# pacificclimate/VIC

Hardware: AMD Instinct MI355X
Metric: cell-timesteps/s (higher is better)
Workload: dtype f64

## Files before the change

vic_amd/csrc/vic_profile.hpp:

```cpp
#pragma once
#include "vic_surface.hpp"

namespace vic {

constexpr int NBUCKET = 2 * (VIC_MID_NODES + 2);
static_assert(NBUCKET <= 64, "one lane per work-list segment when the pending total is summed");

struct PArgs {
  const double* __restrict__ pin;
  const double* __restrict__ ts;
  double* __restrict__ pout;
  const int* __restrict__ pslot;
  const int* __restrict__ list;
  const int* __restrict__ count;
  int cap;
  int* next;
  int* count_zero;
  int* evalonly_zero;
  const int* pend_counts;
  const int* pend_eo;
  int* pend_out;
  int Nn, NOFLUX, EXP_TRANS, TFALLBACK;
  const int* jl;
};

__host__ __device__ inline int pout_stride(int Nn) { return Nn + 1 + (Nn + 1) / 2; }
__host__ __device__ inline int pout_hru_stride(int Nn) { return 2 * pout_stride(Nn) + 2; }
__host__ __device__ inline int pout_key(int Nn, int slot) { return 2 * pout_stride(Nn) + slot; }

constexpr int LOCKSTEP_GATE = 16;

constexpr double NODE_ROOT_RANGE = SOIL_DT + Brent::MAXTRIES * Brent::TSTEP;
constexpr double NODE_NEWTON_TOL = 1.e-8;
constexpr double NODE_PREDICT_TOL2 = 1.e-7;
constexpr int NODE_PREDICT_MAXIT = 12;
constexpr double NODE_NEWTON_ACCEPT = 2.e-11;
constexpr int NODE_NEWTON_MAXIT = 200;

struct NodeK {
  double AT0, B, C, D, EI, S, G, Y, EM, EMM;
  VIC_DEV void load(const double* __restrict__ r) {
    AT0 = r[PR_AT0]; B = r[PR_B]; C = r[PR_C]; D = r[PR_D]; EI = r[PR_EI]; S = r[PR_S]; G = r[PR_G]; Y = r[PR_Y];
    EM = r[PR_EMOIST]; EMM = r[PR_EMM];
// ... 156 lines not shown
    }
  }
  if (ok && !converged) {
    if (TFALLBACK) {
#pragma unroll
      for (int k = 0; k < NN; k++)
        if (k < Nn) { T[k] = T0[k]; cnt_add[k] += 1; }
      fbmask |= (Nn >= 32) ? 0xFFFFFFFFu : ((1u << Nn) - 1u);
    } else ok = false;
  }
}

VIC_DEV int profile_pick(const PArgs& a, const int* bcount, int slot) {
  int rem = slot, found = 0;
#pragma unroll 1
  for (int b = NBUCKET - 1; b >= 0; b--) {
    const int cb = bcount[b];
    if (rem < cb) { found = b * a.cap + rem; break; }
    rem -= cb;
  }
  return a.list[found];
}

constexpr int PROFILE_REG_WAVES = 2;
template <int NN, bool NEWTON>
__global__ __launch_bounds__(64) VIC_WAVES_PER_EU(PROFILE_REG_WAVES, PROFILE_REG_WAVES) void vic_profile_solve_reg(const PArgs a) {
  __shared__ int bcount[NBUCKET];
  __shared__ double T0l[NN * 64];
  __shared__ double Kl[3 * (NN - 2) * 64];
  const int lane = threadIdx.x;
#define T0(j) T0l[(j) * 64 + lane]
#define KL(f, j) Kl[((f) * (NN - 2) + (j) - 1) * 64 + lane]
  for (int b = lane; b < NBUCKET; b += 64) bcount[b] = a.count[b];
  if (blockIdx.x == 0) {
    for (int b = lane; b < NBUCKET; b += 64) a.count_zero[b] = 0;
    if (lane == 0) *a.evalonly_zero = 0;
    int v = (lane < NBUCKET) ? a.pend_counts[lane] : 0;
#pragma unroll
    for (int off = 32; off >= 1; off >>= 1) v += __shfl(v, lane ^ off);
    if (lane == 0) *a.pend_out = v + *a.pend_eo;
  }
  __syncthreads();
  int n = 0;
#pragma unroll
  for (int b = 0; b < NBUCKET; b++) n += bcount[b];
  if ((int)blockIdx.x * 64 >= n) return;

  constexpr int Nn = NN;
  const int jlast = a.NOFLUX ? Nn : Nn - 1;
  const int MAXIT = 1000;
  const double threshold = 1.e-2;
  const bool EXP_TRANS = a.EXP_TRANS != 0;

  bool have = false, sweeping = false, converged = false, ok = true, frozen_on = false;
  int hru = 0, ps = 0, it = 1, jl_lane = 0;
  unsigned fbmask = 0;
  int evcnt = 0;
  double T[NN];
  double kAT0[NN - 1], kB[NN - 1], kC[NN - 1], kD[NN - 1], kEI[NN - 1], kS[NN - 1], kEMM[NN - 1];
#pragma unroll
  for (int k = 0; k < NN; k++) T[k] = 0;
#pragma unroll
  for (int k = 0; k < NN - 1; k++) { kAT0[k] = 0; kB[k] = 0; kC[k] = 0; kD[k] = 0; kEI[k] = 0; kS[k] = 1; kEMM[k] = 0; }
// ... 101 lines not shown
      a.pout[(size_t)hru * pout_hru_stride(Nn) + pout_key(Nn, ps)] = T0(0);
      have = false;
    }
    PROF_ADD(24, t_fin);
  }
#undef T0
#undef KL
}

constexpr int LS_WAVES = 2;
template <int NN, bool NEWTON>
__global__ __launch_bounds__(64) VIC_WAVES_PER_EU(LS_WAVES, LS_WAVES) void vic_profile_solve_lockstep(const PArgs a) {
  using mask_t = typename NodeBound<NN>::mask_t;
  constexpr bool T0_LDS = NN <= VIC_MID_NODES;
  __shared__ int bcount[NBUCKET];
  __shared__ double Tl[NN * 64];
  __shared__ double T0l[T0_LDS ? NN * 64 : 1];
  const int lane = threadIdx.x;
#define T(j) Tl[(j) * 64 + lane]
#define T0(j) (T0_LDS ? T0l[(T0_LDS ? (j) : 0) * 64 + lane] : ((j) == 0 ? T0s : blk[(j) * PREC + PR_T0]))
  for (int b = lane; b < NBUCKET; b += 64) bcount[b] = a.count[b];
  if (blockIdx.x == 0) {
    for (int b = lane; b < NBUCKET; b += 64) a.count_zero[b] = 0;
    if (lane == 0) *a.evalonly_zero = 0;
    int v = (lane < NBUCKET) ? a.pend_counts[lane] : 0;
#pragma unroll
    for (int off = 32; off >= 1; off >>= 1) v += __shfl(v, lane ^ off);
    if (lane == 0) *a.pend_out = v + *a.pend_eo;
  }
  __syncthreads();
  int n = 0;
#pragma unroll
  for (int b = 0; b < NBUCKET; b++) n += bcount[b];
  if ((int)blockIdx.x * 64 >= n) return;

  const int Nn = node_count<NN>(a.Nn);
  const int jlast = a.NOFLUX ? Nn : Nn - 1;
  const int MAXIT = 1000;
  const double threshold = 1.e-2;
  const bool EXP_TRANS = a.EXP_TRANS != 0;

#define LS_REC() (a.pout + (size_t)hru * pout_hru_stride(Nn) + ps * pout_stride(Nn))
#define LS_CNT(j) (reinterpret_cast<int*>(LS_REC() + Nn + 1)[j])
  bool have = false, sweeping = false, converged = false, ok = true, frozen_on = false;
  int hru = 0, ps = 0, it = 1, jl_lane = 0;
  mask_t fbmask = 0;
  const double* __restrict__ blk = a.pin;
  double T0s = 0;
  bool more = true;
  while (true) {
    const unsigned long long idle = __ballot(!have);
// ... 103 lines not shown
```

vic_amd/csrc/vicgpu_api.hip:

```cpp
#include <hip/hip_runtime.h>
#include <stdio.h>
#include <stdlib.h>
#include <string.h>
#include <algorithm>
#include <atomic>
#include <chrono>
#include <memory>
#include <string>
#include <thread>
#include <vector>
#include "vicgpu.h"
#include <cstddef>
#include <type_traits>
#include "vic_glacier.hpp"
#include "vic_profile.hpp"
#include "vic_putdata.hpp"
#include "vic_host.hpp"

using namespace vic;

#define HIPIGN(call) do { hipError_t ign_ = (call); (void)ign_; } while (0)
#define HIPCHK(ctx, call)                                                                              \
  do {                                                                                                 \
    hipError_t e_ = (call);                                                                            \
// ... 42 lines not shown
  Dmy dmy;
  double* sd;
  int* si;
  double* flux;
  int* hru_err;
  const int* glist;
  int gcount;
  unsigned long long* ctx;
  double* pin;
  double* ts;
  double* pout;
  int* pslot;
  int* hstate;
  int* list;
  int* count;
  int list_cap;
  int* hkey;
  double* pimp;
  int* lastexp;
  int* jl;
  int phase;
};

constexpr int CTX_GROUP = 8, CTX_GROUP_B = 2;
constexpr size_t CTX_NA = sizeof(SurfSolve) / 8 + sizeof(SurfEBMut) / 8 + offsetof(SurfEBConst, Cs2) / 8;
constexpr size_t CTX_NA_PAD = (CTX_NA + CTX_GROUP - 1) / CTX_GROUP * CTX_GROUP;
constexpr size_t ctx_padded_words(size_t words) {
  return CTX_NA_PAD + ((words > CTX_NA ? words - CTX_NA : 0) + CTX_GROUP_B - 1) / CTX_GROUP_B * CTX_GROUP_B;
}
struct CtxRef {
  unsigned long long* p;
  int lane;
  VIC_DEV static CtxRef at(unsigned long long* base, size_t words_per_hru, size_t g) {
    return CtxRef{base + (g >> 6) * (ctx_padded_words(words_per_hru) * 64), (int)(g & 63)};
  }
  VIC_DEV unsigned long long* word(size_t W) const {
    if (W < CTX_NA) return p + (W / CTX_GROUP) * (64 * CTX_GROUP) + lane * CTX_GROUP + (W % CTX_GROUP);
    const size_t V = W - CTX_NA;
    return p + CTX_NA_PAD * 64 + (V / CTX_GROUP_B) * (64 * CTX_GROUP_B) + lane * CTX_GROUP_B + (V % CTX_GROUP_B);
  }
};
template <class T>
VIC_DEV void ctx_put(const CtxRef& r, size_t word0, const T& v) {
  static_assert(sizeof(T) % 8 == 0 && std::is_trivially_copyable<T>::value, "context structs are arrays of 8-byte words");
  constexpr int NW = sizeof(T) / 8;
  unsigned long long tmp[NW];
  __builtin_memcpy(tmp, &v, sizeof(T));
#pragma unroll
  for (int i = 0; i < NW; i++) *r.word(word0 + i) = tmp[i];
}
template <class T>
VIC_DEV void ctx_get(const CtxRef& r, size_t word0, T& v) {
  static_assert(sizeof(T) % 8 == 0 && std::is_trivially_copyable<T>::value, "context structs are arrays of 8-byte words");
  constexpr int NW = sizeof(T) / 8;
  unsigned long long tmp[NW];
#pragma unroll
  for (int i = 0; i < NW; i++) tmp[i] = *r.word(word0 + i);
  __builtin_memcpy(&v, tmp, sizeof(T));
}
constexpr int EBC_W_POST = offsetof(SurfEBConst, delta_t) / 8, EBC_W_ALWAYS = offsetof(SurfEBConst, ice0) / 8,
              EBC_W_FROZEN = offsetof(SurfEBConst, kappa_snow) / 8, EBC_W_SNOWCOV = offsetof(SurfEBConst, LongSnowIn) / 8,
              EBC_W_INCL = offsetof(SurfEBConst, lmoist) / 8, EBC_W_EVAP = offsetof(SurfEBConst, Wdew) / 8,
              EBC_W_CANOPY = offsetof(SurfEBConst, Cs2) / 8;
constexpr int EBM_W_FEED = offsetof(SurfEBMut, deltaCC) / 8, EBM_W_IN3 = offsetof(SurfEBMut, Tsnow_surf) / 8,
              EBM_W_TSNOW = offsetof(SurfEBMut, ra_used) / 8, EBM_W_RA1 = EBM_W_TSNOW + 1, EBM_W_VV = offsetof(SurfEBMut, vv) / 8,
              EBM_W_KEEP = offsetof(SurfEBMut, Tnew2) / 8;
static_assert(offsetof(SurfEBMut, fusion) / 8 == EBM_W_IN3 - 1 && offsetof(SurfEBMut, layerevap) / 8 == EBM_W_VV + 3, "SurfEBMut layout");
constexpr size_t CW_SV = sizeof(SurfSolve) / 8, CW_EBM = sizeof(SurfEBMut) / 8, CW_EBC = EBC_W_CANOPY,
                 CW_P = sizeof(SubStep) / 8, CW_L = sizeof(SubLoop) / 8, CW_C = sizeof(StepConst) / 8;
constexpr size_t CO_SV = 0, CO_EBM = CO_SV + CW_SV, CO_EBC = CO_EBM + CW_EBM, CO_P = CO_EBC + CW_EBC, CO_L = CO_P + CW_P,
                 CO_C = CO_L + CW_L, CO_W = CO_C + CW_C;
constexpr size_t CW_W = sizeof(WCarry) / 8, CO_WM = CO_W + CW_W;
template <int NN> constexpr size_t ctx_words() { return CO_WM + sizeof(WCarryMulti<NN>) / 8; }
static_assert(sizeof(StepConstPost) <= sizeof(StepConst), "StepConstPost is parked in StepConst's words");
static_assert(CTX_NA == CO_P, "region A of the context slab = what the evaluation kernel reads");
constexpr size_t CW_L_HEAD = offsetof(SubLoop, st_AlbedoOver) / 8;
constexpr size_t CW_SV_ITER = offsetof(SurfSolve, Tsurf) / 8;

template <class T>
VIC_DEV void ctx_put_words(const CtxRef& r, size_t word0, const T& v, int first, int last) {
  constexpr int NW = sizeof(T) / 8;
#pragma unroll
  for (int i = 0; i < NW; i++)
    if (i >= first && i < last) {
      unsigned long long w;
      __builtin_memcpy(&w, reinterpret_cast<const char*>(&v) + 8 * i, 8);
      *r.word(word0 + i) = w;
    }
}
template <class T>
VIC_DEV void ctx_get_words(const CtxRef& r, size_t word0, T& v, int first, int last) {
  constexpr int NW = sizeof(T) / 8;
#pragma unroll
  for (int i = 0; i < NW; i++)
    if (i >= first && i < last) {
      const unsigned long long w = *r.word(word0 + i);
      __builtin_memcpy(reinterpret_cast<char*>(&v) + 8 * i, &w, 8);
    }
}

// ... 596 lines not shown
  PROF_LANE(1);
}

struct EArgs {
  Opt o;
  LaunchMap map;
  int ncell, nhru, Nn;
  const int* glist;
  int gcount;
  const double* cell_params;
  const int* hpi;
  unsigned long long* ctx;
  size_t ctx_words;
  double* pout;
  int* pslot;
  double* ts;
  int* jl;
  int* hstate;
  int* list_next;
  int* count_next;
  int list_cap;
  const int* hkey;
  int* profile_next;
  int* evalonly;
  int* eo_list_next;
  int list_thr;
  const int* list_cur;
  const int* count_cur;
  const int* eo_list_cur;
  const int* npend_cur;
  int implicit;
  const double* veglib;
  const double* forcing;
  int month;
};

constexpr int EVAL_WAVES = 2;
__global__ __launch_bounds__(64) VIC_WAVES_PER_EU(EVAL_WAVES, EVAL_WAVES) void vic_surf_eval(const EArgs a) {
  if (blockIdx.x == 0 && threadIdx.x == 0) *a.profile_next = 0;
  const int npend = *a.npend_cur;
  int g;
  if (npend <= a.list_thr) {
    if ((int)blockIdx.x * 64 >= npend) return;
    __shared__ int bcount[NBUCKET];
    for (int b = threadIdx.x; b < NBUCKET; b += 64) bcount[b] = a.count_cur[b];
    __syncthreads();
    int nsolve = 0;
#pragma unroll 1
    for (int b = 0; b < NBUCKET; b++) nsolve += bcount[b];
    const int gi = blockIdx.x * 64 + threadIdx.x;
    if (gi >= npend) return;
    if (gi < nsolve) {
      int rem = gi, found = 0;
#pragma unroll 1
      for (int b = 0; b < NBUCKET; b++) {
        const int cb = bcount[b];
        if (rem < cb) { found = b * a.list_cap + rem; break; }
        rem -= cb;
      }
      g = a.list_cur[found];
    } else g = a.eo_list_cur[gi - nsolve];
  } else {
    const int gi = a.map.index(blockIdx.x, threadIdx.x, a.gcount);
    if (gi < 0) return;
    g = a.glist ? a.glist[gi] : gi;
  }
  const int hs = a.hstate[g];
  if ((hs & HS_STATE) != 1) return;
  const int cls = hs >> HS_CLS_SHIFT;
  const size_t nh = a.nhru;
  const int c = a.hpi[(size_t)HPI_CELL * nh + g];
  const int veg_idx = a.hpi[(size_t)HPI_VEG_INDEX * nh + g];
  const int ps = a.pslot[g];
  CellView cv{a.cell_params, a.ncell, c, a.o.Nnode, a.o.Nband};
  const Soil3 s3 = load_soil3(cv);
  SurfSolve sv;
  SurfEB eb;
  const CtxRef cx = CtxRef::at(a.ctx, a.ctx_words, g);
  ctx_get(cx, CO_SV, sv);
  ebc_get(cx, eb, cls);
  const bool is_final = sv.stage == SurfSolve::FINAL;
  const int slot = sv.on_record ? sv.final_slot : ps;
  {
    SurfEBMut& m = eb;
// ... 32 lines not shown
    a.pout[(size_t)g * pout_hru_stride(a.Nn) + pout_key(a.Nn, 1)] = NAN;
  }
  bool need_solve = sv.stage != SurfSolve::DONE;
  if (sv.stage == SurfSolve::FINAL && !a.implicit) {
    if (rec[pout_key(a.Nn, slot)] == sv.x) { sv.final_slot = slot; sv.on_record = 1; need_solve = false; }
    else if (rec[pout_key(a.Nn, slot ^ 1)] == sv.x) { sv.final_slot = slot ^ 1; sv.on_record = 1; need_solve = false; }
  }
  if (sv.stage == stage_before && (sv.stage == SurfSolve::ROOT || sv.stage == SurfSolve::ROOT_QUICK)) ctx_put_words(cx, CO_SV, sv, 0, (int)CW_SV_ITER);
  else ctx_put(cx, CO_SV, sv);
  if (sv.stage == SurfSolve::DONE) {
    const SurfEBMut& m = eb;
    if (at_root) {
      ctx_put_words(cx, CO_EBM, m, EBM_W_KEEP, (int)CW_EBM);
      ctx_put_words(cx, CO_EBM, m, EBM_W_TSNOW, EBM_W_TSNOW + 1);
      if (cls & EBG_FROZEN) ctx_put_words(cx, CO_EBM, m, EBM_W_IN3 - 1, EBM_W_IN3);
      if (cls & EBG_CANOPY) ctx_put_words(cx, CO_EBM, m, EBM_W_VV, EBM_W_VV + 6);
      else if (cls & EBG_EVAP) ctx_put_words(cx, CO_EBM, m, EBM_W_VV + 3, EBM_W_VV + 4);
    } else ctx_put(cx, CO_EBM, m);
  } else if (cls & EBG_INCL) ctx_put_words(cx, CO_EBM, static_cast<const SurfEBMut&>(eb), 0, EBM_W_FEED);
  if (sv.stage == SurfSolve::DONE) a.hstate[g] = 2;
  else if (need_solve) { a.ts[g] = sv.x; a.pslot[g] = slot ^ 1; }
  list_append(a.list_next, a.count_next, a.list_cap, need_solve, a.hkey[g], g);
  {
    const bool eo = sv.stage != SurfSolve::DONE && !need_solve;
    const unsigned long long m = __ballot(eo);
    if (m != 0) {
      const int lane = (int)__lane_id(), lead = __ffsll((long long)m) - 1;
      int base = 0;
      if (lane == lead) base = atomicAdd(a.evalonly, __popcll(m));
      base = __shfl(base, lead);
      if (eo) a.eo_list_next[base + __popcll(m & ((1ull << lane) - 1ull))] = g;
    }
  }
}

struct GArgs {
  Opt o;
  int ncell, nhru, reset;
  const double* cell_params;
  const int* cell_off;
  const int* cell_list;
  const int* hpi;
  double* sd;
  double* eq;
};

__global__ __launch_bounds__(64) void vic_glacier_fit(const GArgs a) {
  const int c = blockIdx.x * 64 + threadIdx.x;
  if (c >= a.ncell) return;
  const size_t nh = a.nhru, nc = a.ncell;
  CellView cv{a.cell_params, a.ncell, c, a.o.Nnode, a.o.Nband};
  double X[VIC_MAX_BANDS], Y[VIC_MAX_BANDS];
  int np = 0;
  for (int k = a.cell_off[c]; k < a.cell_off[c + 1]; k++) {
// ... 269 lines not shown
  I(VICGPU_SR_U(SRU_TFOLIAGE_FBCOUNT, Nn), SI_TFOLIAGE_FBCOUNT); I(VICGPU_SR_U(SRU_TSURF_FBCOUNT, Nn), SI_TSURF_FBCOUNT);
  I(VICGPU_SR_U(SRU_GLAC_SURF_TEMP_FBCOUNT, Nn), SI_GLAC_SURF_TEMP_FBCOUNT); I(VICGPU_SR_U(SRU_SNOW_SURF_TEMP_FBCOUNT, Nn), SI_SNOW_SURF_TEMP_FBCOUNT);
  I(VICGPU_SR_U(SRU_GLAC_SURF_TEMP_FBFLAG, Nn), SI_GLAC_SURF_TEMP_FBFLAG);
  F(VICGPU_SR_U(SRU_GLAC_VAPOR_FLUX, Nn), FX_GLAC_VAPOR_FLUX);
  if (GATHER) r[VICGPU_SR_U(SRU_SNOW_CANOPY_ALBEDO, Nn)] = 0.0;
  F(VICGPU_SR_U(SRU_SNOW_SURFACE_FLUX, Nn), FX_SNOW_SURFACE_FLUX);
  I(VICGPU_SR_U(SRU_SNOW_SURF_TEMP_FBFLAG, Nn), SI_SNOW_SURF_TEMP_FBFLAG);
  D(VICGPU_SR_U(SRU_SNOW_TMP_INT_STORAGE, Nn), SD_SNOW_TMP_INT_STORAGE);
  F(VICGPU_SR_U(SRU_SNOW_VAPOR_FLUX, Nn), FX_SNOW_VAPOR_FLUX);
#undef D
#undef I
#undef F
}

constexpr int RB_LAG = 3, RB_DEPTH = RB_LAG + 1;
struct FdChunk {
  int c0 = 0, ccount = 0;
  DevBuf<int> d_glist;
  int gcount = 0;
  LaunchMap map;
  DevBuf<int> d_list[2];
  DevBuf<int> d_fb_list, d_fb_count;
  DevBuf<int> d_count;
  DevBuf<int> d_elist[2];
  int list_cap = 0;
  PinnedBuf<int> h_count;
  Stream stream;
  Event done, readback[RB_DEPTH];
  std::string err;
  int status = 0;
  long long rounds = 0, steps = 0;
};

struct Domain {
  int ncell = 0, nhru = 0;
  bool domain_ready = false;
  bool any_glacier = false;
  DevBuf<double> d_cp, d_hpd, d_sd, d_flux, d_cell_out, d_accum;
  DevBuf<int> d_hpi, d_si, d_cell_off, d_cell_list, d_hru_err, d_cell_err;
  bool fd = false;
  DevBuf<unsigned long long> d_ctx;
  DevBuf<double> d_pin, d_ts, d_pout;
  DevBuf<int> d_hstate, d_pslot, d_hkey, d_lastexp, d_jl;
  DevBuf<double> d_pimp;
  std::vector<FdChunk> chunks;
  bool put_on = false;
  int out_nrow = 0;
  OutLayout out_lay;
// ... 10 lines not shown
  DevBuf<double> d_veglib;
  Domain dom;
  double* d_forcing = nullptr;
  unsigned char* d_snowflag = nullptr;
  std::vector<int> dmy;
  int chunk_steps = 0;
  struct ForcingSlot {
    DevBuf<double> d_f, d_raw;
    DevBuf<unsigned char> d_s;
    PinnedBuf<char> h_stage;
    std::vector<int> dmy;
    int nsteps = 0;
    Event uploaded;
    Event released;
    bool upload_pending = false, was_current = false;
  } slot[2];
  int cur = -1, staged = -1;
  Stream stream, copy_stream;
  std::vector<Event> ev;
  int ev_used = 0;
  int write_fluxes = 1;
  int steps_done = 0;
  int profile_waves = 0;
  int eval_list_pct = 30;
  bool node_newton = false;
  int ev_steps = 0;
  int out_step_ratio = 1;
};

static void free_domain(vicgpu_ctx* c) {
  c->dom = Domain();
  c->chunk_steps = 0;
  c->dmy.clear();
  c->cur = c->staged = -1;
  c->d_forcing = nullptr; c->d_snowflag = nullptr;
}

template <int NN>
static hipError_t launch_hru(const KArgs& ka, hipStream_t st, bool ordinary, bool glacier) {
  const int nblk = ka.map.nblocks(ka.gcount);
  if constexpr (NN == 3) {
    if (ordinary) hipLaunchKernelGGL((vic_hru_step<NN, false>), dim3(nblk), dim3(64), 0, st, ka);
  }
  if (glacier) hipLaunchKernelGGL((vic_hru_step<NN, true>), dim3(nblk), dim3(64), 0, st, ka);
  return hipGetLastError();
}

// ... 19 lines not shown
  if constexpr (NN == 10) {
    if (newton) hipLaunchKernelGGL((vic_profile_solve_reg<NN, true>), g, b, 0, st, pa);
    else hipLaunchKernelGGL((vic_profile_solve_reg<NN, false>), g, b, 0, st, pa);
  } else {
    if (newton) hipLaunchKernelGGL((vic_profile_solve_lockstep<NN, true>), g, b, 0, st, pa);
    else hipLaunchKernelGGL((vic_profile_solve_lockstep<NN, false>), g, b, 0, st, pa);
  }
  return hipGetLastError();
}

template <int NN>
static int profile_resident_waves(int device, bool newton) {
  int per_cu = 0, ncu = 0;
  hipError_t e;
  if constexpr (NN == 10) e = newton ? hipOccupancyMaxActiveBlocksPerMultiprocessor(&per_cu, vic_profile_solve_reg<NN, true>, 64, 0)
                                     : hipOccupancyMaxActiveBlocksPerMultiprocessor(&per_cu, vic_profile_solve_reg<NN, false>, 64, 0);
  else e = newton ? hipOccupancyMaxActiveBlocksPerMultiprocessor(&per_cu, vic_profile_solve_lockstep<NN, true>, 64, 0)
                  : hipOccupancyMaxActiveBlocksPerMultiprocessor(&per_cu, vic_profile_solve_lockstep<NN, false>, 64, 0);
  if (e != hipSuccess || per_cu <= 0) per_cu = 8;
  if (hipDeviceGetAttribute(&ncu, hipDeviceAttributeMultiprocessorCount, device) != hipSuccess || ncu <= 0) ncu = 256;
  return per_cu * ncu;
}

constexpr int CNT_LIST_STRIDE = 64, CNT_CURSOR = 128, CNT_EVALONLY = 160, CNT_EVALONLY_STRIDE = 32, CNT_NPEND = 224, CNT_TOTAL = 256;
static_assert(NBUCKET <= CNT_LIST_STRIDE, "counter block layout");
static inline int* cnt_list(int* d_count, int l) { return d_count + l * CNT_LIST_STRIDE; }
static inline int* cnt_evalonly(int* d_count, int l) { return d_count + CNT_EVALONLY + l * CNT_EVALONLY_STRIDE; }

static int fd_read_count(FdChunk* ch, int which, int* nsolve, int* nevalonly) {
  HIPCHK(ch, hipMemcpyAsync(ch->h_count, ch->d_count, sizeof(int) * CNT_TOTAL, hipMemcpyDeviceToHost, ch->stream));
  HIPCHK(ch, hipStreamSynchronize(ch->stream));
  int n = 0;
  for (int b = 0; b < NBUCKET; b++) n += ch->h_count[which * CNT_LIST_STRIDE + b];
  *nsolve = n;
  *nevalonly = ch->h_count[CNT_EVALONLY + which * CNT_EVALONLY_STRIDE];
  return VICGPU_OK;
}

#define NODE_DISPATCH(Nnode, F, ...)                                                                                          \
  (node_bound(Nnode) == 10 ? F<10>(__VA_ARGS__)                                                                           \
                           : node_bound(Nnode) == VIC_MID_NODES ? F<VIC_MID_NODES>(__VA_ARGS__) : F<VIC_MAX_NODES>(__VA_ARGS__))

static int fd_step(vicgpu_ctx* c, FdChunk* ch, KArgs ka) {
  const int Nn = c->o.Nnode;
  hipStream_t st = ch->stream;
  if (c->dom.any_glacier) HIPCHK(ch, NODE_DISPATCH(Nn, launch_hru, ka, st, false, true));
  HIPCHK(ch, hipMemsetAsync(ch->d_count, 0, sizeof(int) * CNT_TOTAL, st));
  int cur = 0;
  ka.phase = 0; ka.list = ch->d_list[cur]; ka.count = cnt_list(ch->d_count, cur); ka.list_cap = ch->list_cap;
  HIPCHK(ch, NODE_DISPATCH(Nn, launch_fd_stage, ka, c->o.NF > 1, st));
  PArgs pa;
  pa.pin = c->dom.d_pin; pa.ts = c->dom.d_ts; pa.pout = c->dom.d_pout; pa.pslot = c->dom.d_pslot; pa.Nn = Nn; pa.NOFLUX = c->o.NOFLUX; pa.EXP_TRANS = c->o.EXP_TRANS;
  pa.TFALLBACK = c->o.TFALLBACK; pa.next = ch->d_count + CNT_CURSOR; pa.cap = ch->list_cap; pa.jl = c->dom.d_jl;
  EArgs ea;
  ea.o = c->o; ea.ncell = c->dom.ncell; ea.nhru = c->dom.nhru; ea.Nn = Nn; ea.glist = ch->d_glist; ea.gcount = ch->gcount; ea.map = ch->map;
  ea.cell_params = c->dom.d_cp; ea.hpi = c->dom.d_hpi; ea.ctx = c->dom.d_ctx;
  ea.ctx_words = NODE_DISPATCH(Nn, ctx_words);
  ea.pout = c->dom.d_pout; ea.pslot = c->dom.d_pslot; ea.ts = c->dom.d_ts; ea.hstate = c->dom.d_hstate; ea.profile_next = ch->d_count + CNT_CURSOR;
  ea.list_thr = (int)((long long)ch->gcount * c->eval_list_pct / 100);
  ea.list_cap = ch->list_cap; ea.hkey = c->dom.d_hkey; ea.implicit = c->o.IMPLICIT; ea.jl = c->dom.d_jl;
  ea.veglib = c->d_veglib; ea.forcing = ka.forcing; ea.month = ka.dmy.month;
  const bool trace_rounds = getenv("VICGPU_TRACE_ROUNDS") != nullptr;
  const int FREE_ROUNDS = 6;
  const int nsub = c->o.NF;
  for (int p = 1; p <= nsub; p++) {
    int nmax = ch->gcount;
    int npend = -1;
    int rb_list[RB_DEPTH];
    int rb_first = -1;
    for (int round = 0;; round++) {
      pa.list = ch->d_list[cur]; pa.count = cnt_list(ch->d_count, cur); pa.count_zero = cnt_list(ch->d_count, cur ^ 1);
      pa.evalonly_zero = cnt_evalonly(ch->d_count, cur ^ 1);
      pa.pend_counts = cnt_list(ch->d_count, cur); pa.pend_eo = cnt_evalonly(ch->d_count, cur); pa.pend_out = ch->d_count + CNT_NPEND;
      if (c->o.IMPLICIT) {
        HIPCHK(ch, hipMemsetAsync(ch->d_fb_count, 0, sizeof(int) * (NBUCKET + 1), st));
        IArgs ia;
        ia.ncell = c->dom.ncell; ia.nhru = c->dom.nhru; ia.Nband = c->o.Nband; ia.pimp = c->dom.d_pimp; ia.hpi = c->dom.d_hpi; ia.cell_params = c->dom.d_cp;
        ia.hkey = c->dom.d_hkey; ia.fb_list = ch->d_fb_list; ia.fb_count = ch->d_fb_count; ia.lastexp = c->dom.d_lastexp; ia.cursor = ch->d_fb_count + NBUCKET;
        {
          int nblk = (nmax + 63) / 64;
          if (nblk > 4096) nblk = 4096;
          if (nblk < 1) nblk = 1;
          hipLaunchKernelGGL(vic_profile_solve_implicit, dim3(nblk), dim3(64), 0, st, pa, ia);
        }
        HIPCHK(ch, hipGetLastError());
        pa.list = ch->d_fb_list; pa.count = ch->d_fb_count;
      }
      HIPCHK(ch, NODE_DISPATCH(Nn, launch_profile, pa, nmax, c->profile_waves, c->node_newton, st));
      ea.list_next = ch->d_list[cur ^ 1]; ea.count_next = cnt_list(ch->d_count, cur ^ 1);
      ea.evalonly = cnt_evalonly(ch->d_count, cur ^ 1); ea.eo_list_next = ch->d_elist[cur ^ 1];
      ea.list_cur = ch->d_list[cur]; ea.count_cur = cnt_list(ch->d_count, cur);
      ea.eo_list_cur = ch->d_elist[cur]; ea.npend_cur = ch->d_count + CNT_NPEND;
      const bool sparse = npend >= 0 && npend <= ea.list_thr;
      hipLaunchKernelGGL(vic_surf_eval, dim3(sparse ? ((npend + 63) / 64 > 0 ? (npend + 63) / 64 : 1) : ea.map.nblocks(ch->gcount)), dim3(64), 0, st, ea);
      HIPCHK(ch, hipGetLastError());
      cur ^= 1;
      ch->rounds++;
      if (trace_rounds) {
        int n = 0, ne = 0;
        if (fd_read_count(ch, cur, &n, &ne) != VICGPU_OK) return VICGPU_ERR_HIP;
        fprintf(stderr, "vicgpu rounds: chunk %d sub-step %d round %d leaves %d solves + %d evaluation-only of %d\n", (int)(ch - &c->dom.chunks[0]), p, round, n, ne, ch->gcount);
      }
      if (round + 2 >= FREE_ROUNDS) {
        const int slot = round % RB_DEPTH;
        if (rb_first < 0) rb_first = round;
        HIPCHK(ch, hipMemcpyAsync(ch->h_count + slot * CNT_TOTAL, ch->d_count, sizeof(int) * CNT_TOTAL, hipMemcpyDeviceToHost, st));
        HIPCHK(ch, hipEventRecord(ch->readback[slot], st));
        rb_list[slot] = cur;
      }
      if (rb_first >= 0 && round - RB_LAG >= rb_first) {
        const int slot = (round - RB_LAG) % RB_DEPTH;
        HIPCHK(ch, hipEventSynchronize(ch->readback[slot]));
        const int* h = ch->h_count + slot * CNT_TOTAL;
        int n = 0;
        for (int b = 0; b < NBUCKET; b++) n += h[rb_list[slot] * CNT_LIST_STRIDE + b];
        const int neo = h[CNT_EVALONLY + rb_list[slot] * CNT_EVALONLY_STRIDE];
        if (n == 0 && neo == 0) break;
        nmax = n;
        npend = n + neo;
      }
    }
    ka.phase = p; ka.list = ch->d_list[cur]; ka.count = cnt_list(ch->d_count, cur);
    HIPCHK(ch, NODE_DISPATCH(Nn, launch_fd_stage, ka, c->o.NF > 1, st));
    if (p < nsub) {
      int n = 0, ne = 0;
      const int r = fd_read_count(ch, cur, &n, &ne);
      if (r != VICGPU_OK) return r;
      if (n == 0) break;
    }
  }
  ch->steps++;
  return VICGPU_OK;
}

static hipError_t launch_put_data(const vicgpu_ctx* c, hipStream_t st, int c0, int ccount, int s) {
  OArgs a;
  a.o = c->o; a.lay = c->dom.out_lay; a.ncell = c->dom.ncell; a.nhru = c->dom.nhru; a.c0 = c0; a.ccount = ccount;
  a.rec = s < 0 ? -1 : 0; a.out_step_ratio = c->out_step_ratio;
  a.cell_off = c->dom.d_cell_off; a.cell_list = c->dom.d_cell_list; a.cell_params = c->dom.d_cp; a.veglib = c->d_veglib;
  a.hpi = c->dom.d_hpi; a.hpd = c->dom.d_hpd; a.sd = c->dom.d_sd; a.si = c->dom.d_si; a.flux = c->dom.d_flux;
  a.forcing = s < 0 ? nullptr : c->d_forcing + (size_t)s * VIC_NFORCE * (c->o.NR + 1) * c->dom.ncell;
  a.cell_out = c->dom.d_cell_out; a.out_data = c->dom.d_out_data; a.out_agg = c->dom.d_out_agg; a.pb = c->dom.d_pb;
// ... 231 lines not shown
      ch.c0 = (int)((long long)ncell * k / nchunk);
      ch.ccount = (int)((long long)ncell * (k + 1) / nchunk) - ch.c0;
      std::vector<int> gl(cell_hru_list + cell_hru_offset[ch.c0], cell_hru_list + cell_hru_offset[ch.c0 + ch.ccount]);
      std::sort(gl.begin(), gl.end());
      ch.gcount = (int)gl.size();
      ch.map = LaunchMap();
      if (ch.ccount > 0 && ch.gcount % ch.ccount == 0 && !getenv("VICGPU_NO_XCD_MAP")) {
        const int nslot = ch.gcount / ch.ccount;
        bool regular = true;
        for (int sl = 0; sl < nslot && regular; sl++)
          for (int i = 0; i < ch.ccount; i++)
            if (gl[(size_t)sl * ch.ccount + i] != sl * ncell + ch.c0 + i || hpi[(size_t)HPI_CELL * nhru + gl[(size_t)sl * ch.ccount + i]] != ch.c0 + i) {
              regular = false;
              break;
            }
        if (regular) { ch.map.nslot = nslot; ch.map.ccount = ch.ccount; }
      }
      const size_t gn = ch.gcount > 0 ? ch.gcount : 1;
      HIPCHK(c, ch.d_glist.alloc(gn));
      ch.list_cap = ch.gcount > 0 ? ch.gcount : 1;
      HIPCHK(c, ch.d_list[0].alloc(gn * NBUCKET));
      HIPCHK(c, ch.d_list[1].alloc(gn * NBUCKET));
      HIPCHK(c, ch.d_count.alloc(CNT_TOTAL));
      HIPCHK(c, ch.d_elist[0].alloc(gn));
      HIPCHK(c, ch.d_elist[1].alloc(gn));
      if (c->o.IMPLICIT) {
        HIPCHK(c, ch.d_fb_list.alloc(gn * NBUCKET));
        HIPCHK(c, ch.d_fb_count.alloc(NBUCKET + 1));
      }
      HIPCHK(c, ch.h_count.alloc((size_t)CNT_TOTAL * RB_DEPTH));
      if (ch.gcount) HIPCHK(c, copy_on(c->stream, ch.d_glist, gl.data(), sizeof(int) * ch.gcount, hipMemcpyHostToDevice));
      HIPCHK(c, ch.stream.create());
      HIPCHK(c, ch.done.create(hipEventDisableTiming));
      for (Event& e : ch.readback) HIPCHK(c, e.create(hipEventDisableTiming));
    }
  }
  return VICGPU_OK;
}

int vicgpu_set_domain(vicgpu_ctx* c, int ncell, int nhru, const double* cell_params, const int* hpi, const double* hpd,
                      const int* cell_hru_offset, const int* cell_hru_list) {
  if (!c) return VICGPU_ERR_ARG;
  const int r = set_domain_impl(c, ncell, nhru, cell_params, hpi, hpd, cell_hru_offset, cell_hru_list);
  if (r == VICGPU_OK) c->dom.domain_ready = true;
  else if (r == VICGPU_ERR_HIP || r == VICGPU_ERR_NOMEM) {
    HIPIGN(hipSetDevice(c->device));
    free_domain(c);
  }
// ... 623 lines not shown
```

Measured before the change: 3.853 million.

## Stripe pending-HRU work list and regroup context slab by access class

Replaces the single global evaluation-only counter and split solve/eval-only lookup with a single pending list spread over 64 per-block stripes. The profile kernel builds a prefix sum over the stripe counts, and the sparse evaluation kernel finds each entry by binary search. This is meant to reduce atomic contention on one counter and simplify index lookup. It also permutes the region-A context words so that fields read together sit in the same sectors. The sparse-list threshold rises from 30% to 75% and is disabled in round 0. Costs include more counter memory, a larger host readback and a 64-entry reduction on the host.

```diff
diff --git a/vic_amd/csrc/vic_profile.hpp b/vic_amd/csrc/vic_profile.hpp
--- a/vic_amd/csrc/vic_profile.hpp
+++ b/vic_amd/csrc/vic_profile.hpp
@@ -5,6 +5,7 @@
 
 constexpr int NBUCKET = 2 * (VIC_MID_NODES + 2);
 static_assert(NBUCKET <= 64, "one lane per work-list segment when the pending total is summed");
+constexpr int PEND_STRIPES = 64, PEND_CNT_STRIDE = 32;
 
 struct PArgs {
   const double* __restrict__ pin;
@@ -16,9 +17,10 @@
   int cap;
   int* next;
   int* count_zero;
-  int* evalonly_zero;
   const int* pend_counts;
-  const int* pend_eo;
+  const int* pend_stripes;
+  int* pend_stripes_zero;
+  int* pend_prefix;
   int* pend_out;
   int Nn, NOFLUX, EXP_TRANS, TFALLBACK;
   const int* jl;
@@ -221,6 +223,22 @@
   return a.list[found];
 }
 
+static_assert(PEND_STRIPES == 64, "one lane per stripe");
+VIC_DEV void pend_pack(const PArgs& a, int lane, int keyed_total) {
+  a.pend_stripes_zero[lane * PEND_CNT_STRIDE] = 0;
+  const int cnt = a.pend_stripes[lane * PEND_CNT_STRIDE];
+  int incl = cnt;
+#pragma unroll
+  for (int off = 1; off < 64; off <<= 1) {
+    const int up = __shfl(incl, lane >= off ? lane - off : lane);
+    if (lane >= off) incl += up;
+  }
+  a.pend_prefix[lane + 1] = incl;
+  if (lane == 0) a.pend_prefix[0] = 0;
+  const int total = __shfl(incl, 63);
+  if (lane == 0) *a.pend_out = total > 0 ? total : keyed_total;
+}
+
 constexpr int PROFILE_REG_WAVES = 2;
 template <int NN, bool NEWTON>
 __global__ __launch_bounds__(64) VIC_WAVES_PER_EU(PROFILE_REG_WAVES, PROFILE_REG_WAVES) void vic_profile_solve_reg(const PArgs a) {
@@ -233,11 +251,10 @@
   for (int b = lane; b < NBUCKET; b += 64) bcount[b] = a.count[b];
   if (blockIdx.x == 0) {
     for (int b = lane; b < NBUCKET; b += 64) a.count_zero[b] = 0;
-    if (lane == 0) *a.evalonly_zero = 0;
     int v = (lane < NBUCKET) ? a.pend_counts[lane] : 0;
 #pragma unroll
     for (int off = 32; off >= 1; off >>= 1) v += __shfl(v, lane ^ off);
-    if (lane == 0) *a.pend_out = v + *a.pend_eo;
+    pend_pack(a, lane, v);
   }
   __syncthreads();
   int n = 0;
@@ -385,11 +402,10 @@
   for (int b = lane; b < NBUCKET; b += 64) bcount[b] = a.count[b];
   if (blockIdx.x == 0) {
     for (int b = lane; b < NBUCKET; b += 64) a.count_zero[b] = 0;
-    if (lane == 0) *a.evalonly_zero = 0;
     int v = (lane < NBUCKET) ? a.pend_counts[lane] : 0;
 #pragma unroll
     for (int off = 32; off >= 1; off >>= 1) v += __shfl(v, lane ^ off);
-    if (lane == 0) *a.pend_out = v + *a.pend_eo;
+    pend_pack(a, lane, v);
   }
   __syncthreads();
   int n = 0;
diff --git a/vic_amd/csrc/vicgpu_api.hip b/vic_amd/csrc/vicgpu_api.hip
--- a/vic_amd/csrc/vicgpu_api.hip
+++ b/vic_amd/csrc/vicgpu_api.hip
@@ -88,42 +88,6 @@
   int phase;
 };
 
-constexpr int CTX_GROUP = 8, CTX_GROUP_B = 2;
-constexpr size_t CTX_NA = sizeof(SurfSolve) / 8 + sizeof(SurfEBMut) / 8 + offsetof(SurfEBConst, Cs2) / 8;
-constexpr size_t CTX_NA_PAD = (CTX_NA + CTX_GROUP - 1) / CTX_GROUP * CTX_GROUP;
-constexpr size_t ctx_padded_words(size_t words) {
-  return CTX_NA_PAD + ((words > CTX_NA ? words - CTX_NA : 0) + CTX_GROUP_B - 1) / CTX_GROUP_B * CTX_GROUP_B;
-}
-struct CtxRef {
-  unsigned long long* p;
-  int lane;
-  VIC_DEV static CtxRef at(unsigned long long* base, size_t words_per_hru, size_t g) {
-    return CtxRef{base + (g >> 6) * (ctx_padded_words(words_per_hru) * 64), (int)(g & 63)};
-  }
-  VIC_DEV unsigned long long* word(size_t W) const {
-    if (W < CTX_NA) return p + (W / CTX_GROUP) * (64 * CTX_GROUP) + lane * CTX_GROUP + (W % CTX_GROUP);
-    const size_t V = W - CTX_NA;
-    return p + CTX_NA_PAD * 64 + (V / CTX_GROUP_B) * (64 * CTX_GROUP_B) + lane * CTX_GROUP_B + (V % CTX_GROUP_B);
-  }
-};
-template <class T>
-VIC_DEV void ctx_put(const CtxRef& r, size_t word0, const T& v) {
-  static_assert(sizeof(T) % 8 == 0 && std::is_trivially_copyable<T>::value, "context structs are arrays of 8-byte words");
-  constexpr int NW = sizeof(T) / 8;
-  unsigned long long tmp[NW];
-  __builtin_memcpy(tmp, &v, sizeof(T));
-#pragma unroll
-  for (int i = 0; i < NW; i++) *r.word(word0 + i) = tmp[i];
-}
-template <class T>
-VIC_DEV void ctx_get(const CtxRef& r, size_t word0, T& v) {
-  static_assert(sizeof(T) % 8 == 0 && std::is_trivially_copyable<T>::value, "context structs are arrays of 8-byte words");
-  constexpr int NW = sizeof(T) / 8;
-  unsigned long long tmp[NW];
-#pragma unroll
-  for (int i = 0; i < NW; i++) tmp[i] = *r.word(word0 + i);
-  __builtin_memcpy(&v, tmp, sizeof(T));
-}
 constexpr int EBC_W_POST = offsetof(SurfEBConst, delta_t) / 8, EBC_W_ALWAYS = offsetof(SurfEBConst, ice0) / 8,
               EBC_W_FROZEN = offsetof(SurfEBConst, kappa_snow) / 8, EBC_W_SNOWCOV = offsetof(SurfEBConst, LongSnowIn) / 8,
               EBC_W_INCL = offsetof(SurfEBConst, lmoist) / 8, EBC_W_EVAP = offsetof(SurfEBConst, Wdew) / 8,
@@ -139,9 +103,95 @@
 constexpr size_t CW_W = sizeof(WCarry) / 8, CO_WM = CO_W + CW_W;
 template <int NN> constexpr size_t ctx_words() { return CO_WM + sizeof(WCarryMulti<NN>) / 8; }
 static_assert(sizeof(StepConstPost) <= sizeof(StepConst), "StepConstPost is parked in StepConst's words");
-static_assert(CTX_NA == CO_P, "region A of the context slab = what the evaluation kernel reads");
 constexpr size_t CW_L_HEAD = offsetof(SubLoop, st_AlbedoOver) / 8;
 constexpr size_t CW_SV_ITER = offsetof(SurfSolve, Tsurf) / 8;
+
+constexpr int CTX_GROUP = 8, CTX_GROUP_B = 2;
+constexpr size_t CTX_NA = sizeof(SurfSolve) / 8 + sizeof(SurfEBMut) / 8 + offsetof(SurfEBConst, Cs2) / 8;
+static_assert(CTX_NA == CO_P, "region A of the context slab = what the evaluation kernel reads");
+constexpr int CTXR_ITER = 0, CTXR_COMMON = 16, CTXR_CLASS = 48, CTXR_SNOW = 64, CTXR_COLD = 72, CTXR_END = 104;
+struct CtxMap { unsigned char slab[CTX_NA]; int end[6]; };
+constexpr int ctx_map_run(CtxMap& m, int at, size_t first, size_t last) {
+  for (size_t w = first; w < last; w++) m.slab[w] = (unsigned char)at++;
+  return at;
+}
+constexpr CtxMap ctx_make_map() {
+  CtxMap m{};
+  int at = ctx_map_run(m, CTXR_ITER, CO_SV, CO_SV + CW_SV_ITER);
+  m.end[0] = at;
+  at = ctx_map_run(m, CTXR_COMMON, CO_EBM + EBM_W_FEED, CO_EBM + EBM_W_TSNOW);
+  at = ctx_map_run(m, at, CO_EBM + EBM_W_RA1, CO_EBM + EBM_W_RA1 + 1);
+  at = ctx_map_run(m, at, CO_EBC, CO_EBC + EBC_W_ALWAYS);
+  m.end[1] = at;
+  at = ctx_map_run(m, CTXR_CLASS, CO_EBC + EBC_W_ALWAYS, CO_EBC + EBC_W_FROZEN);
+  at = ctx_map_run(m, at, CO_EBC + EBC_W_INCL, CO_EBC + EBC_W_CANOPY);
+  m.end[2] = at;
+  at = ctx_map_run(m, CTXR_SNOW, CO_EBC + EBC_W_FROZEN, CO_EBC + EBC_W_INCL);
+  m.end[3] = at;
+  at = ctx_map_run(m, CTXR_COLD, CO_SV + CW_SV_ITER, CO_SV + CW_SV);
+  m.end[4] = at;
+  at = ctx_map_run(m, at, CO_EBM + EBM_W_TSNOW, CO_EBM + EBM_W_TSNOW + 1);
+  at = ctx_map_run(m, at, CO_EBM, CO_EBM + EBM_W_FEED);
+  at = ctx_map_run(m, at, CO_EBM + EBM_W_VV, CO_EBM + CW_EBM);
+  m.end[5] = at;
+  return m;
+}
+constexpr CtxMap CTX_MAP = ctx_make_map();
+constexpr bool ctx_map_is_permutation() {
+  bool used[CTXR_END] = {};
+  for (size_t w = 0; w < CTX_NA; w++) {
+    if (CTX_MAP.slab[w] >= CTXR_END || used[CTX_MAP.slab[w]]) return false;
+    used[CTX_MAP.slab[w]] = true;
+  }
+  int n = 0;
+  for (int i = 0; i < CTXR_END; i++) n += used[i] ? 1 : 0;
+  return n == (int)CTX_NA;
+}
+static_assert(ctx_map_is_permutation(), "parking map of region A");
+static_assert(CTXR_ITER % CTX_GROUP == 0 && CTXR_COMMON % CTX_GROUP == 0 && CTXR_CLASS % CTX_GROUP == 0 && CTXR_SNOW % CTX_GROUP == 0
+              && CTXR_COLD % CTX_GROUP == 0 && CTXR_END % CTX_GROUP == 0, "every range of the parking map starts on a sector boundary");
+static_assert(CTX_MAP.end[0] == CTXR_COMMON && CTX_MAP.end[1] <= CTXR_CLASS && CTX_MAP.end[2] <= CTXR_SNOW && CTX_MAP.end[3] <= CTXR_COLD
+              && CTX_MAP.end[4] <= CTXR_COLD + CTX_GROUP && CTX_MAP.end[5] <= CTXR_END && CTXR_END - CTX_MAP.end[5] < CTX_GROUP,
+              "ranges of the parking map; the tail of SurfSolve, which every evaluation fetches, in one sector");
+static_assert(CTX_MAP.end[1] - CTXR_COMMON == 31 && CTX_MAP.end[2] - CTXR_CLASS == 13,
+              "the iteration's inputs: 4 sectors for every class, 2 more for frozen soil / evaporation / canopy");
+constexpr size_t CTX_NA_PAD = CTXR_END;
+constexpr size_t ctx_padded_words(size_t words) {
+  return CTX_NA_PAD + ((words > CTX_NA ? words - CTX_NA : 0) + CTX_GROUP_B - 1) / CTX_GROUP_B * CTX_GROUP_B;
+}
+struct CtxRef {
+  unsigned long long* p;
+  int lane;
+  VIC_DEV static CtxRef at(unsigned long long* base, size_t words_per_hru, size_t g) {
+    return CtxRef{base + (g >> 6) * (ctx_padded_words(words_per_hru) * 64), (int)(g & 63)};
+  }
+  VIC_DEV unsigned long long* word(size_t W) const {
+    if (W < CTX_NA) {
+      const size_t S = CTX_MAP.slab[W];
+      return p + (S / CTX_GROUP) * (64 * CTX_GROUP) + lane * CTX_GROUP + (S % CTX_GROUP);
+    }
+    const size_t V = W - CTX_NA;
+    return p + CTX_NA_PAD * 64 + (V / CTX_GROUP_B) * (64 * CTX_GROUP_B) + lane * CTX_GROUP_B + (V % CTX_GROUP_B);
+  }
+};
+template <class T>
+VIC_DEV void ctx_put(const CtxRef& r, size_t word0, const T& v) {
+  static_assert(sizeof(T) % 8 == 0 && std::is_trivially_copyable<T>::value, "context structs are arrays of 8-byte words");
+  constexpr int NW = sizeof(T) / 8;
+  unsigned long long tmp[NW];
+  __builtin_memcpy(tmp, &v, sizeof(T));
+#pragma unroll
+  for (int i = 0; i < NW; i++) *r.word(word0 + i) = tmp[i];
+}
+template <class T>
+VIC_DEV void ctx_get(const CtxRef& r, size_t word0, T& v) {
+  static_assert(sizeof(T) % 8 == 0 && std::is_trivially_copyable<T>::value, "context structs are arrays of 8-byte words");
+  constexpr int NW = sizeof(T) / 8;
+  unsigned long long tmp[NW];
+#pragma unroll
+  for (int i = 0; i < NW; i++) tmp[i] = *r.word(word0 + i);
+  __builtin_memcpy(&v, tmp, sizeof(T));
+}
 
 template <class T>
 VIC_DEV void ctx_put_words(const CtxRef& r, size_t word0, const T& v, int first, int last) {
@@ -784,12 +834,12 @@
   int list_cap;
   const int* hkey;
   int* profile_next;
-  int* evalonly;
-  int* eo_list_next;
+  int* pend_list_next;
+  int* pend_count_next;
+  int pend_cap;
   int list_thr;
-  const int* list_cur;
-  const int* count_cur;
-  const int* eo_list_cur;
+  const int* pend_list_cur;
+  const int* pend_prefix;
   const int* npend_cur;
   int implicit;
   const double* veglib;
@@ -804,24 +854,19 @@
   int g;
   if (npend <= a.list_thr) {
     if ((int)blockIdx.x * 64 >= npend) return;
-    __shared__ int bcount[NBUCKET];
-    for (int b = threadIdx.x; b < NBUCKET; b += 64) bcount[b] = a.count_cur[b];
+    __shared__ int prefix[PEND_STRIPES + 1];
+    for (int b = threadIdx.x; b < PEND_STRIPES + 1; b += 64) prefix[b] = a.pend_prefix[b];
     __syncthreads();
-    int nsolve = 0;
-#pragma unroll 1
-    for (int b = 0; b < NBUCKET; b++) nsolve += bcount[b];
     const int gi = blockIdx.x * 64 + threadIdx.x;
     if (gi >= npend) return;
-    if (gi < nsolve) {
-      int rem = gi, found = 0;
-#pragma unroll 1
-      for (int b = 0; b < NBUCKET; b++) {
-        const int cb = bcount[b];
-        if (rem < cb) { found = b * a.list_cap + rem; break; }
-        rem -= cb;
-      }
-      g = a.list_cur[found];
-    } else g = a.eo_list_cur[gi - nsolve];
+    int lo = 0, hi = PEND_STRIPES;
+#pragma unroll
+    for (int it = 0; it < 6; it++) {
+      const int mid = (lo + hi) >> 1;
+      const bool up = prefix[mid] <= gi;
+      lo = up ? mid : lo; hi = up ? hi : mid;
+    }
+    g = a.pend_list_cur[(size_t)lo * a.pend_cap + (gi - prefix[lo])];
   } else {
     const int gi = a.map.index(blockIdx.x, threadIdx.x, a.gcount);
     if (gi < 0) return;
@@ -900,14 +945,14 @@
   else if (need_solve) { a.ts[g] = sv.x; a.pslot[g] = slot ^ 1; }
   list_append(a.list_next, a.count_next, a.list_cap, need_solve, a.hkey[g], g);
   {
-    const bool eo = sv.stage != SurfSolve::DONE && !need_solve;
-    const unsigned long long m = __ballot(eo);
+    const bool pend = sv.stage != SurfSolve::DONE;
+    const unsigned long long m = __ballot(pend);
     if (m != 0) {
-      const int lane = (int)__lane_id(), lead = __ffsll((long long)m) - 1;
+      const int lane = (int)__lane_id(), lead = __ffsll((long long)m) - 1, stripe = blockIdx.x % PEND_STRIPES;
       int base = 0;
-      if (lane == lead) base = atomicAdd(a.evalonly, __popcll(m));
+      if (lane == lead) base = atomicAdd(a.pend_count_next + stripe * PEND_CNT_STRIDE, __popcll(m));
       base = __shfl(base, lead);
-      if (eo) a.eo_list_next[base + __popcll(m & ((1ull << lane) - 1ull))] = g;
+      if (pend) a.pend_list_next[(size_t)stripe * a.pend_cap + base + __popcll(m & ((1ull << lane) - 1ull))] = g;
     }
   }
 }
@@ -1223,8 +1268,9 @@
   DevBuf<int> d_list[2];
   DevBuf<int> d_fb_list, d_fb_count;
   DevBuf<int> d_count;
-  DevBuf<int> d_elist[2];
+  DevBuf<int> d_plist[2];
   int list_cap = 0;
+  int pend_cap = 0;
   PinnedBuf<int> h_count;
   Stream stream;
   Event done, readback[RB_DEPTH];
@@ -1281,7 +1327,7 @@
   int write_fluxes = 1;
   int steps_done = 0;
   int profile_waves = 0;
-  int eval_list_pct = 30;
+  int eval_list_pct = 75;
   bool node_newton = false;
   int ev_steps = 0;
   int out_step_ratio = 1;
@@ -1347,18 +1393,24 @@
   return per_cu * ncu;
 }
 
-constexpr int CNT_LIST_STRIDE = 64, CNT_CURSOR = 128, CNT_EVALONLY = 160, CNT_EVALONLY_STRIDE = 32, CNT_NPEND = 224, CNT_TOTAL = 256;
-static_assert(NBUCKET <= CNT_LIST_STRIDE, "counter block layout");
+constexpr int CNT_LIST_STRIDE = 64, CNT_CURSOR = 128, CNT_NPEND = 160, CNT_PREFIX = 192, CNT_STRIPES = 288,
+              CNT_STRIPES_STRIDE = PEND_STRIPES * PEND_CNT_STRIDE, CNT_TOTAL = CNT_STRIPES + 2 * CNT_STRIPES_STRIDE;
+static_assert(NBUCKET <= CNT_LIST_STRIDE && CNT_PREFIX + PEND_STRIPES + 1 <= CNT_STRIPES && CNT_STRIPES % 32 == 0, "counter block layout");
 static inline int* cnt_list(int* d_count, int l) { return d_count + l * CNT_LIST_STRIDE; }
-static inline int* cnt_evalonly(int* d_count, int l) { return d_count + CNT_EVALONLY + l * CNT_EVALONLY_STRIDE; }
-
-static int fd_read_count(FdChunk* ch, int which, int* nsolve, int* nevalonly) {
+static inline int* cnt_stripes(int* d_count, int l) { return d_count + CNT_STRIPES + l * CNT_STRIPES_STRIDE; }
+static inline int cnt_pending(const int* h_count, int l) {
+  int n = 0;
+  for (int s = 0; s < PEND_STRIPES; s++) n += h_count[CNT_STRIPES + l * CNT_STRIPES_STRIDE + s * PEND_CNT_STRIDE];
+  return n;
+}
+
+static int fd_read_count(FdChunk* ch, int which, int* nsolve, int* npending) {
   HIPCHK(ch, hipMemcpyAsync(ch->h_count, ch->d_count, sizeof(int) * CNT_TOTAL, hipMemcpyDeviceToHost, ch->stream));
   HIPCHK(ch, hipStreamSynchronize(ch->stream));
   int n = 0;
   for (int b = 0; b < NBUCKET; b++) n += ch->h_count[which * CNT_LIST_STRIDE + b];
   *nsolve = n;
-  *nevalonly = ch->h_count[CNT_EVALONLY + which * CNT_EVALONLY_STRIDE];
+  *npending = cnt_pending(ch->h_count, which);
   return VICGPU_OK;
 }
 
@@ -1382,7 +1434,8 @@
   ea.cell_params = c->dom.d_cp; ea.hpi = c->dom.d_hpi; ea.ctx = c->dom.d_ctx;
   ea.ctx_words = NODE_DISPATCH(Nn, ctx_words);
   ea.pout = c->dom.d_pout; ea.pslot = c->dom.d_pslot; ea.ts = c->dom.d_ts; ea.hstate = c->dom.d_hstate; ea.profile_next = ch->d_count + CNT_CURSOR;
-  ea.list_thr = (int)((long long)ch->gcount * c->eval_list_pct / 100);
+  const int list_thr = (int)((long long)ch->gcount * c->eval_list_pct / 100);
+  ea.pend_cap = ch->pend_cap;
   ea.list_cap = ch->list_cap; ea.hkey = c->dom.d_hkey; ea.implicit = c->o.IMPLICIT; ea.jl = c->dom.d_jl;
   ea.veglib = c->d_veglib; ea.forcing = ka.forcing; ea.month = ka.dmy.month;
   const bool trace_rounds = getenv("VICGPU_TRACE_ROUNDS") != nullptr;
@@ -1395,8 +1448,8 @@
     int rb_first = -1;
     for (int round = 0;; round++) {
       pa.list = ch->d_list[cur]; pa.count = cnt_list(ch->d_count, cur); pa.count_zero = cnt_list(ch->d_count, cur ^ 1);
-      pa.evalonly_zero = cnt_evalonly(ch->d_count, cur ^ 1);
-      pa.pend_counts = cnt_list(ch->d_count, cur); pa.pend_eo = cnt_evalonly(ch->d_count, cur); pa.pend_out = ch->d_count + CNT_NPEND;
+      pa.pend_counts = cnt_list(ch->d_count, cur); pa.pend_stripes = cnt_stripes(ch->d_count, cur);
+      pa.pend_stripes_zero = cnt_stripes(ch->d_count, cur ^ 1); pa.pend_prefix = ch->d_count + CNT_PREFIX; pa.pend_out = ch->d_count + CNT_NPEND;
       if (c->o.IMPLICIT) {
         HIPCHK(ch, hipMemsetAsync(ch->d_fb_count, 0, sizeof(int) * (NBUCKET + 1), st));
         IArgs ia;
@@ -1413,18 +1466,18 @@
       }
       HIPCHK(ch, NODE_DISPATCH(Nn, launch_profile, pa, nmax, c->profile_waves, c->node_newton, st));
       ea.list_next = ch->d_list[cur ^ 1]; ea.count_next = cnt_list(ch->d_count, cur ^ 1);
-      ea.evalonly = cnt_evalonly(ch->d_count, cur ^ 1); ea.eo_list_next = ch->d_elist[cur ^ 1];
-      ea.list_cur = ch->d_list[cur]; ea.count_cur = cnt_list(ch->d_count, cur);
-      ea.eo_list_cur = ch->d_elist[cur]; ea.npend_cur = ch->d_count + CNT_NPEND;
+      ea.pend_list_next = ch->d_plist[cur ^ 1]; ea.pend_count_next = cnt_stripes(ch->d_count, cur ^ 1);
+      ea.pend_list_cur = ch->d_plist[cur]; ea.pend_prefix = ch->d_count + CNT_PREFIX; ea.npend_cur = ch->d_count + CNT_NPEND;
+      ea.list_thr = round > 0 ? list_thr : -1;
       const bool sparse = npend >= 0 && npend <= ea.list_thr;
       hipLaunchKernelGGL(vic_surf_eval, dim3(sparse ? ((npend + 63) / 64 > 0 ? (npend + 63) / 64 : 1) : ea.map.nblocks(ch->gcount)), dim3(64), 0, st, ea);
       HIPCHK(ch, hipGetLastError());
       cur ^= 1;
       ch->rounds++;
       if (trace_rounds) {
-        int n = 0, ne = 0;
-        if (fd_read_count(ch, cur, &n, &ne) != VICGPU_OK) return VICGPU_ERR_HIP;
-        fprintf(stderr, "vicgpu rounds: chunk %d sub-step %d round %d leaves %d solves + %d evaluation-only of %d\n", (int)(ch - &c->dom.chunks[0]), p, round, n, ne, ch->gcount);
+        int n = 0, np = 0;
+        if (fd_read_count(ch, cur, &n, &np) != VICGPU_OK) return VICGPU_ERR_HIP;
+        fprintf(stderr, "vicgpu rounds: chunk %d sub-step %d round %d leaves %d solves + %d evaluation-only of %d\n", (int)(ch - &c->dom.chunks[0]), p, round, n, np - n, ch->gcount);
       }
       if (round + 2 >= FREE_ROUNDS) {
         const int slot = round % RB_DEPTH;
@@ -1439,10 +1492,10 @@
         const int* h = ch->h_count + slot * CNT_TOTAL;
         int n = 0;
         for (int b = 0; b < NBUCKET; b++) n += h[rb_list[slot] * CNT_LIST_STRIDE + b];
-        const int neo = h[CNT_EVALONLY + rb_list[slot] * CNT_EVALONLY_STRIDE];
-        if (n == 0 && neo == 0) break;
+        const int np = cnt_pending(h, rb_list[slot]);
+        if (np == 0) break;
         nmax = n;
-        npend = n + neo;
+        npend = np;
       }
     }
     ka.phase = p; ka.list = ch->d_list[cur]; ka.count = cnt_list(ch->d_count, cur);
@@ -1720,8 +1773,10 @@
       HIPCHK(c, ch.d_list[0].alloc(gn * NBUCKET));
       HIPCHK(c, ch.d_list[1].alloc(gn * NBUCKET));
       HIPCHK(c, ch.d_count.alloc(CNT_TOTAL));
-      HIPCHK(c, ch.d_elist[0].alloc(gn));
-      HIPCHK(c, ch.d_elist[1].alloc(gn));
+      ch.pend_cap = 64 * ((ch.map.nblocks(ch.gcount) + PEND_STRIPES - 1) / PEND_STRIPES);
+      if (ch.pend_cap < 64) ch.pend_cap = 64;
+      HIPCHK(c, ch.d_plist[0].alloc((size_t)ch.pend_cap * PEND_STRIPES));
+      HIPCHK(c, ch.d_plist[1].alloc((size_t)ch.pend_cap * PEND_STRIPES));
       if (c->o.IMPLICIT) {
         HIPCHK(c, ch.d_fb_list.alloc(gn * NBUCKET));
         HIPCHK(c, ch.d_fb_count.alloc(NBUCKET + 1));
```

Result: faster. 3.935 million (median of 6 runs) (+2.1%).
